# barry-mir/mixing-style-transfer

Hardware: AMD Instinct MI355X
Metric: triplets/sec (10 s @ 44.1 kHz, 4-stem, bs=24) (higher is better)
Workload: dtype f32

## Files before the change

### mixing-style-transfer_amd/csrc/fft_pk.h

```cpp
#pragma once
#include <hip/hip_runtime.h>

namespace mstpk {

typedef float v2f __attribute__((ext_vector_type(2)));
typedef float v4f __attribute__((ext_vector_type(4)));

__device__ __forceinline__ v2f mk(float x, float y) {
  v2f r;
  r.x = x, r.y = y;
  return r;
}
__device__ __forceinline__ v2f add_mi(v2f a, v2f b) {
  v2f d;
  asm("v_pk_add_f32 %0, %1, %2 op_sel:[0,1] op_sel_hi:[1,0] neg_hi:[0,1]" : "=v"(d) : "v"(a), "v"(b));
  return d;
}
__device__ __forceinline__ v2f sub_mi(v2f a, v2f b) {
  v2f d;
  asm("v_pk_add_f32 %0, %1, %2 op_sel:[0,1] op_sel_hi:[1,0] neg_lo:[0,1]" : "=v"(d) : "v"(a), "v"(b));
  return d;
}
__device__ __forceinline__ v2f cmul(v2f a, v2f w) {
  v2f t, d;
// ... 32 lines not shown
  v[2] = add_mi(e2, o2);
  v[6] = sub_mi(e2, o2);
  v[3] = add_mi(e3, o3);
  v[7] = sub_mi(e3, o3);
}

__device__ __forceinline__ void dft16(v2f* x) {
  constexpr float c1 = 0.92387953251128675613f, s1 = 0.38268343236508977173f;
#pragma unroll
  for (int a = 0; a < 4; ++a) dft4(x[a], x[a + 4], x[a + 8], x[a + 12]);
  x[1 + 4] = cmul(x[1 + 4], mk(c1, -s1));
  x[1 + 8] = mul_w8(x[1 + 8]);
  x[1 + 12] = cmul(x[1 + 12], mk(s1, -c1));
  x[2 + 4] = mul_w8(x[2 + 4]);
  x[2 + 12] = mul_w8(x[2 + 12]);
  x[3 + 4] = cmul(x[3 + 4], mk(s1, -c1));
  x[3 + 8] = mul_w8(x[3 + 8]);
  x[3 + 12] = cmul(x[3 + 12], mk(-c1, s1));
  dft4(x[0], x[1], x[2], x[3]);
  dft4(x[4], x[5], x[6], x[7]);
  dft4<true, true>(x[8], x[9], x[10], x[11]);
  dft4<true, false>(x[12], x[13], x[14], x[15]);
}

constexpr int kScr = 1152;
constexpr int kTw2Rows = 7;
constexpr int kTw3Rows = 14;

__device__ __forceinline__ int jb_of(int lane) { return lane ? 128 - lane : 64; }

struct NoFill {
  __device__ __forceinline__ void operator()() const {}
};
template <class F1 = NoFill, class F2 = NoFill>
__device__ __forceinline__ void fft1024(v2f (&x)[16], v2f* scr, const v2f* tw2, const v2f* tw3, int lane, F1 fill1 = F1(),
                                        F2 fill2 = F2()) {
  dft16(x);
  {
    v4f* row = reinterpret_cast<v4f*>(scr + 18 * lane);
#pragma unroll
    for (int q = 0; q < 8; ++q) {
      v4f w;
      w.x = x[2 * q].x, w.y = x[2 * q].y, w.z = x[2 * q + 1].x, w.w = x[2 * q + 1].y;
      row[q] = w;
    }
  }
  __builtin_amdgcn_wave_barrier();
  {
    const int m = lane & 15;
    const v2f* src = scr + 18 * (lane >> 4) + (m >> 2) + 4 * (m & 3);
#pragma unroll
    for (int u = 0; u < 2; ++u)
#pragma unroll
      for (int t = 0; t < 8; ++t) x[8 * u + t] = src[72 * u + 144 * t];
    v2f w2[8];
#pragma unroll
    for (int t = 1; t < 8; ++t) w2[t] = tw2[(t - 1) * 64 + lane];
    fill1();
#pragma unroll
    for (int t = 1; t < 8; ++t) {
      x[t] = cmul(x[t], w2[t]);
      x[8 + t] = cmul(x[8 + t], w2[t]);
    }
    dft8(x);
    dft8(x + 8);
  }
  __builtin_amdgcn_wave_barrier();
  {
    v2f* dst = scr + 144 * (lane >> 4) + (lane & 15);
#pragma unroll
    for (int u = 0; u < 2; ++u)
#pragma unroll
      for (int t = 0; t < 8; ++t) dst[576 * u + 16 * t] = x[8 * u + t];
  }
  __builtin_amdgcn_wave_barrier();
  {
    const v2f* sa = scr + lane;
    const v2f* sb = scr + jb_of(lane);
#pragma unroll
    for (int t = 0; t < 8; ++t) x[t] = sa[144 * t], x[8 + t] = sb[144 * t];
    fill2();
#pragma unroll
    for (int t = 1; t < 8; ++t) {
      x[t] = cmul(x[t], tw3[(t - 1) * 64 + lane]);
      x[8 + t] = cmul(x[8 + t], tw3[(7 + t - 1) * 64 + lane]);
    }
    dft8(x);
    dft8(x + 8);
  }
}

inline void fill_twiddles_host(float2* tw2, float2* tw3) {
  const double pi = 3.14159265358979323846;
  for (int t = 1; t < 8; ++t)
    for (int lane = 0; lane < 64; ++lane) {
      const double a = -2.0 * pi * (double)((lane & 15) * t) / 128.0;
      tw2[(t - 1) * 64 + lane] = make_float2((float)cos(a), (float)sin(a));
      for (int u = 0; u < 2; ++u) {
        const int j = u ? (lane ? 128 - lane : 64) : lane;
        const double b = -2.0 * pi * (double)(j * t) / 1024.0;
        tw3[(u * 7 + t - 1) * 64 + lane] = make_float2((float)cos(b), (float)sin(b));
      }
    }
}

}
```

### mixing-style-transfer_amd/csrc/melfeat.hip

```cpp
#include "common.h"
#include "fft_wave.h"
#include "fft_pk.h"
#include "stage_a_tables.h"

#include <algorithm>
#include <cmath>
#include <memory>
#include <vector>


namespace {

constexpr int kWaves = 8;
constexpr int kFPW = 2;
constexpr int kTF = kWaves * kFPW;
constexpr int kTileStride = kTF + 1;
constexpr int kThreads = kWaves * 64;
constexpr int nf_of(int n_fft) { return n_fft >= 2048 ? 1 : kFPW; }
constexpr int kNumScalars = 80;

enum : int {
  S_LOGSUM = 0,
  S_LINSUM = 4,
  S_MASK = 8,
// ... 970 lines not shown
}

template <int NFFT, int NB, typename ST>
int launch_melfeat(const KParams& kp, int grid, hipStream_t st) {
  return launch_stage_a<melfeat_kernel<NFFT, NB, ST>>(kp, grid, kThreads, GenericLds<NFFT>::bytes(kp.tw_count, kp.tw2_count, kp.nnz, kp.M, kp.tile_bufs), st);
}
template <int NFFT, typename ST, int WPS>
int launch_melfeat_spw(const KParams& kp, int grid, hipStream_t st) {
  return launch_stage_a<melfeat_spw_kernel<NFFT, ST, WPS>>(kp, grid, SpwGeom<WPS>::THREADS, SpwLds<NFFT, WPS>::bytes(kp.tw2_count, kp.nnz, kp.M), st);
}

#include "melfeat_v2.inc"
#include "melfeat_v2_2048.inc"

}

static_assert(sizeof(stage_a::F2) == sizeof(float2), "stage_a_tables.h's pairs are uploaded as float2");

struct mst_plan {
  int sr, n_fft, hop, n_mels, detailed_bins, feat_dim;
  int batches_per_run;
  mst::DevBuf<float> window;
  struct {
    int nb, nnz, tw_count, tw2_count, glen[4], goff[4];
    mst::DevBuf<float2> tw, tw2, post;
    mst::DevBuf<float> melw;
    mst::DevBuf<LaneBand> lanebands;
  } gen;
  struct {
    bool ok = false;
    int wps = 3;
    int nslot = 0, maxcnt = 0, segw_count = 0, glen[kV2Slots] = {0}, goff[kV2Slots] = {0};
    mst::DevBuf<float2> tw2, tw3, tw4, segw;
    mst::DevBuf<int> start, id, bandtab;
  } sw;
};

namespace {

struct StageAEnv {
  int batches_per_run, spw_wps;
  bool v2_wps2, generic, v2_nostd;
  bool old_kernels;
};
StageAEnv read_stage_a_env() {
  auto num = [](const char* name, int dflt) { const char* e = getenv(name); return e ? atoi(e) : dflt; };
  const char* a = getenv("MST_STAGE_A");
  StageAEnv s;
  s.batches_per_run = getenv("MST_MELFEAT_BATCHES") ? std::max(1, num("MST_MELFEAT_BATCHES", 0)) : 0;
  s.spw_wps = num("MST_SPW_WPS", 3);
  s.v2_wps2 = num("MST_V2_WPS", 0) == 2, s.generic = getenv("MST_MELFEAT_GENERIC"), s.v2_nostd = getenv("MST_V2_NOSTD");
  s.old_kernels = s.generic || (a && (!strcmp(a, "spw") || !strcmp(a, "generic")));
  return s;
}

int frames_per_run_of(const mst_plan* p, int F) {
  if (p->batches_per_run > 0) return p->batches_per_run * kTF;
  int fpr = (F + 31) / 32;
  fpr += fpr & 1;
  return std::max(2 * kTF, fpr);
}
int runs_per_clip(const mst_plan* p, int F) {
  const int fpr = frames_per_run_of(p, F);
  return (F + fpr - 1) / fpr;
}
int pstride_of(const mst_plan* p) { return 4 * p->n_mels + kNumScalars; }
// ... 22 lines not shown
  MST_REQUIRE(hop >= 1 && n_mels >= 4 && n_mels <= 256, "mst_plan_create: bad hop=%d / n_mels=%d", hop, n_mels);
  MST_REQUIRE(detailed_bins >= 0 && detailed_bins <= 256 && (detailed_bins == 0 || detailed_bins < n_mels ||
              detailed_bins == n_mels), "mst_plan_create: bad detailed_bins=%d", detailed_bins);
  std::unique_ptr<mst_plan> p(new mst_plan());
  p->sr = sample_rate, p->n_fft = n_fft, p->hop = hop, p->n_mels = n_mels, p->detailed_bins = detailed_bins;
  const int sd = detailed_bins > 0 ? detailed_bins + 2 : 5;
  p->feat_dim = 4 * (10 + sd) + 4;
  const StageAEnv env = read_stage_a_env();
  p->batches_per_run = env.batches_per_run;
  const int n_bins = n_fft / 2 + 1;
  auto& g = p->gen;
  auto& sw = p->sw;
  const bool v2 = n_fft == 1024 && hop == 256, v4 = n_fft == 2048 && hop == 512 && n_mels <= 128;
  sw.wps = (env.v2_wps2 || n_mels > 128 || v4) ? 2 : 3;
  stage_a::PieceTable t;
  if (v2 || v4) t = stage_a::build_pieces(fb, n_bins, n_mels, v2 ? stage_a::v2_piece_opts(n_mels) : stage_a::v4_piece_opts());
  sw.ok = t.ok, sw.nslot = t.nslot, sw.maxcnt = t.maxcnt, sw.segw_count = (int)t.segw.size();
  for (int r = 0; r < kV2Slots; ++r) sw.glen[r] = t.glen[r], sw.goff[r] = t.goff[r];
  const std::vector<int> bands = !t.ok ? std::vector<int>() : v2 ? stage_a::pack_bands16(t, n_mels, stage_a::kV2Dump) : stage_a::pack_bands8(t, n_mels);
  std::vector<float2> t2(mstpk::kTw2Rows * 64), t3(mstpk::kTw3Rows * 64);
  mstpk::fill_twiddles_host(t2.data(), t3.data());
  const std::vector<stage_a::F2> t4 = v4 ? stage_a::tw4_twiddles() : std::vector<stage_a::F2>();

  g.nb = n_mels <= 128 ? 2 : 4;
  const stage_a::LaneBandTable lb = stage_a::build_lane_bands(fb, n_bins, n_mels, g.nb);
  g.nnz = lb.nnz;
  for (int r = 0; r < 4; ++r) g.glen[r] = lb.glen[r], g.goff[r] = lb.goff[r];
  const std::vector<stage_a::F2> tw = stage_a::fft_twiddles(n_fft / 2), post = stage_a::post_twiddles(n_fft);
  std::vector<stage_a::F2> tw2;
  if (n_fft <= 1024) tw2 = stage_a::fft_twiddles(n_fft);
  g.tw_count = (int)tw.size(), g.tw2_count = (int)tw2.size();
  if (tw2.empty()) tw2.push_back(stage_a::F2{1.f, 0.f});
  auto f2 = [](const std::vector<stage_a::F2>& v) { return reinterpret_cast<const float2*>(v.data()); };
  int rc;
  if ((t.ok && ((rc = sw.tw2.upload(t2.data(), t2.size())) || (rc = sw.tw3.upload(t3.data(), t3.size())) ||
                (v4 && (rc = sw.tw4.upload(f2(t4), t4.size()))) || (rc = sw.segw.upload(f2(t.segw), t.segw.size())) ||
                (rc = sw.start.upload(t.start.data(), t.start.size())) || (rc = sw.id.upload(t.id.data(), t.id.size())) ||
                (rc = sw.bandtab.upload(bands.data(), bands.size())))) ||
      (rc = p->window.upload(window, (size_t)n_fft)) || (rc = g.tw.upload(f2(tw), tw.size())) || (rc = g.tw2.upload(f2(tw2), tw2.size())) ||
      (rc = g.post.upload(f2(post), post.size())) || (rc = g.melw.upload(lb.melw.data(), lb.melw.size())) ||
      (rc = g.lanebands.upload(lb.lanebands.data(), lb.lanebands.size())))
    return rc;
  *out = p.release();
  return MST_OK;
}

void mst_plan_destroy(mst_plan* p) { delete p; }

int mst_plan_frames(const mst_plan* p, int T) { return p ? 1 + T / p->hop : MST_EINVAL; }
int mst_plan_feature_dim(const mst_plan* p) { return p ? p->feat_dim : MST_EINVAL; }

size_t mst_melfeat_workspace_bytes(const mst_plan* p, int B, int T) {
  if (!p || B <= 0 || T <= 0) return 0;
  const int F = 1 + T / p->hop;
  const int runs = std::max(runs_per_clip(p, F), p->sw.ok ? sw_runs(p, F) : 0);
  return mst::align_up((size_t)B * runs * pstride_of(p) * sizeof(float), 256);
}

}

namespace {

struct LogmelOut {
  int layout = MST_LOGMEL_REF;
  void* lo = nullptr;
  unsigned* absmax = nullptr;
};

bool plan_uses_v2(const mst_plan* p) { return p->sw.ok && !read_stage_a_env().old_kernels; }

template <typename Fn>
int with_sample_type(bool pcm16, Fn fn) { return pcm16 ? fn(short{}) : fn(float{}); }
template <typename Fn>
auto with_n_fft(int n_fft, Fn fn) {
  if (n_fft == 512) return fn(std::integral_constant<int, 512>{});
  if (n_fft == 1024) return fn(std::integral_constant<int, 1024>{});
  return fn(std::integral_constant<int, 2048>{});
}

template <typename Params, typename Launch>
int launch_sliding_window(const mst_plan* p, Params& k, const LogmelOut& lmo, bool pcm16, Launch launch) {
  const auto& sw = p->sw;
  k.out_mode = lmo.layout, k.logmel_lo = lmo.lo, k.absmax = lmo.absmax;
  k.tw2 = sw.tw2.get(), k.tw3 = sw.tw3.get(), k.segw = sw.segw.get();
  k.nslot = sw.nslot, k.segw_count = sw.segw_count, k.maxcnt = sw.maxcnt, k.fpw = sw_fpw(p, k.F);
  for (size_t r = 0; r < std::size(k.glen); ++r) k.glen[r] = sw.glen[r], k.goff[r] = sw.goff[r];
  return with_sample_type(pcm16, launch);
}

int launch_v2_2048(const mst_plan* p, K4Params k, const LogmelOut& lmo, bool pcm16, hipStream_t st) {
  k.tw4 = p->sw.tw4.get(), k.pstart = p->sw.start.get(), k.pid = p->sw.id.get(), k.bandtab = p->sw.bandtab.get();
  return launch_sliding_window(p, k, lmo, pcm16, [&](auto s) { return launch_melfeat_v2_2048<decltype(s)>(k, k.B * k.runs_per_clip, st); });
}

int launch_v2(const mst_plan* p, K2Params k, const LogmelOut& lmo, bool pcm16, bool no_std, hipStream_t st) {
  k.segstart = p->sw.start.get(), k.segid = p->sw.id.get(), k.bandtab = reinterpret_cast<const int2*>(p->sw.bandtab.get());
  const bool stdt = v2_table_is_standard(p) && !no_std;
  return launch_sliding_window(p, k, lmo, pcm16, [&](auto s) {
    using ST = decltype(s);
    const int grid = k.B * k.runs_per_clip;
    if (p->n_mels > 128) return launch_melfeat_v2<ST, 2, 4>(k, grid, st);
    return p->sw.wps == 3 ? launch_melfeat_v2<ST, 3>(k, grid, st, stdt) : launch_melfeat_v2<ST, 2>(k, grid, st);
  });
}

size_t generic_lds_bytes(const mst_plan* p, int tile_bufs) {
  return with_n_fft(p->n_fft, [&](auto N) { return GenericLds<N()>::bytes(p->gen.tw_count, p->gen.tw2_count, p->gen.nnz, p->n_mels, tile_bufs); });
}

int launch_generic_or_spw(const mst_plan* p, KParams kp, bool pcm16, const StageAEnv& env, hipStream_t st) {
  const auto& g = p->gen;
  kp.tw = g.tw.get(), kp.tw2 = g.tw2.get(), kp.post = g.post.get(), kp.melw = g.melw.get(), kp.lanebands = g.lanebands.get();
  kp.hop = p->hop, kp.tw_count = g.tw_count, kp.tw2_count = g.tw2_count, kp.nnz = g.nnz;
  for (int r = 0; r < 4; ++r) kp.glen[r] = g.glen[r], kp.goff[r] = g.goff[r];
  kp.frames_per_run = frames_per_run_of(p, kp.F);
  bool base16 = true;
  for (int i = 0; i < 4; ++i) base16 = base16 && (reinterpret_cast<uintptr_t>(kp.stem[i]) & 15) == 0;
  kp.vec_ok = base16 && (kp.T % 2 == 0) && (p->hop % 2 == 0) && (kp.clip_stride % 2 == 0);
  kp.vec4_ok = base16 && (kp.T % 4 == 0) && (p->hop % 4 == 0) && (kp.clip_stride % 4 == 0);
  kp.tile_bufs = generic_lds_bytes(p, 2) <= kMaxLds ? 2 : 1;
  const int grid = kp.B * kp.runs_per_clip, n_fft = p->n_fft, M = p->n_mels;
  const bool spw_ok = kp.vec_ok && kp.vec4_ok && p->hop * 4 == n_fft && M <= 128 && g.nb == 2 && (n_fft == 512 || n_fft == 1024) && !env.generic;
  const bool spw3 = spw_ok && env.spw_wps == 3 && n_fft == 1024 && SpwLds<1024, 3>::bytes(g.tw2_count, g.nnz, M) <= kMaxLds;
  const bool spw2 = spw_ok && !spw3 &&
                    (n_fft == 1024 ? SpwLds<1024, 2>::bytes(g.tw2_count, g.nnz, M) : SpwLds<512, 2>::bytes(g.tw2_count, g.nnz, M)) <= kMaxLds;
  return with_sample_type(pcm16, [&](auto s) {
    using ST = decltype(s);
    if (spw3) return launch_melfeat_spw<1024, ST, 3>(kp, grid, st);
    if (spw2) return n_fft == 1024 ? launch_melfeat_spw<1024, ST, 2>(kp, grid, st) : launch_melfeat_spw<512, ST, 2>(kp, grid, st);
// ... 102 lines not shown
```

### mixing-style-transfer_amd/csrc/melfeat_v2.inc

```

constexpr int kV2Slots = 6;

struct K2Params {
  const void* stem[4];
  long long clip_stride;
  float* logmel;
  void* logmel_lo;
  unsigned* absmax;
  int out_mode;
  float* partials;
  const float* window;
  const float2* tw2;
  const float2* tw3;
  const float2* segw;
  const int* segstart;
  const int* segid;
  const int2* bandtab;
  int B, T, F, M;
  int nslot, glen[kV2Slots], goff[kV2Slots], segw_count;
  int maxcnt;
  int fpw;
  int runs_per_clip, pstride;
};

namespace v2 {
using namespace mstpk;

constexpr int kP2 = 0;
constexpr int kExN = 288;
constexpr int kExDump = kExN - 1;
constexpr int kExHi = 544;
constexpr int kExLo = kExHi + kExN;
static_assert(kExLo + kExN <= kScr, "exchange areas must fit the FFT scratch");
static_assert(kExDump == stage_a::kV2Dump && kV2Slots == stage_a::kMaxSlots, "the piece table is built for these limits");

__device__ __forceinline__ v2f pair_power4(v2f zk, v2f zm) {
  const v2f s = zk + zm, d = zk - zm;
  const v2f q = s * s;
  v2f r;
  asm("v_pk_fma_f32 %0, %1, %1, %2 op_sel:[1,1,0] op_sel_hi:[0,0,1]" : "=v"(r) : "v"(d), "v"(q));
  return r;
}

__device__ __forceinline__ v2f sel2(unsigned long long m, v2f a, v2f b) {
  float rx, ry;
  const float ax = a.x, ay = a.y, bx = b.x, by = b.y;
  asm("v_cndmask_b32 %0, %1, %2, %3" : "=v"(rx) : "v"(bx), "v"(ax), "s"(m));
  asm("v_cndmask_b32 %0, %1, %2, %3" : "=v"(ry) : "v"(by), "v"(ay), "s"(m));
  return mk(rx, ry);
}

template <typename ST>
__device__ __forceinline__ float ld_at(const ST* base, int idx) {
  const unsigned boff = (unsigned)idx * (unsigned)sizeof(ST);
  return Smp<ST>::lds(reinterpret_cast<const ST*>(reinterpret_cast<const char*>(base) + boff));
}

__device__ __forceinline__ v2f bcast_fma(float w, v2f q, v2f acc) { return __builtin_elementwise_fma(mk(w, w), q, acc); }

typedef float f4u __attribute__((ext_vector_type(4), aligned(4)));

typedef float f32x4v __attribute__((ext_vector_type(4)));
typedef _Float16 h16x2 __attribute__((ext_vector_type(2)));

template <int NBL>
struct CmGeom {
  static constexpr int MB = 64 * NBL, PSTR = 2 * MB + 16, TILE = 4 * PSTR;
};
template <int NBL, int BLK>
__device__ __forceinline__ void block_absmax(const float (&out)[2 * NBL][BLK], int lane, int nv, int M, unsigned* s_amax) {
  float bm = 0.f;
#pragma unroll
  for (int r = 0; r < NBL; ++r)
#pragma unroll
    for (int e = 0; e < BLK; ++e)
      if (e < nv && lane + 64 * r < M) bm = fmaxf(bm, fmaxf(fabsf(out[2 * r][e]), fabsf(out[2 * r + 1][e])));
  bm = mst::wave_max(bm);
  if (lane == 0) atomicMax(s_amax, __float_as_uint(bm));
}
template <int NBL, int BLK, int WPS, int SCR>
__device__ __forceinline__ void cm_stage(const float (&out)[2 * NBL][BLK], v2f* s_scr, int h, int stem, int lane, int nv, int out_mode) {
  using G = CmGeom<NBL>;
  static_assert((BLK / 4) * G::TILE <= 2 * SCR, "the staged frames of a wave must fit its FFT scratch");
#pragma unroll
  for (int e = 0; e < BLK; ++e) {
    if (e < nv) {
      float* tl = reinterpret_cast<float*>(s_scr + ((e & 3) * WPS + h) * SCR) + (e >> 2) * G::TILE + stem * G::PSTR;
#pragma unroll
      for (int r = 0; r < NBL; ++r) {
        const float vL = out[2 * r][e], vR = out[2 * r + 1][e];
        v2f val;
// ... 36 lines not shown
          const int b = 64 * it + lane;
          v2f a[4];
#pragma unroll
          for (int j = 0; j < 4; ++j) a[j] = *reinterpret_cast<const v2f*>(tl + j * G::PSTR + 2 * b);
          if (b < M) {
            dhi[b] = f32x4v{a[0].x, a[1].x, a[2].x, a[3].x};
            if (logmel_lo) dlo[b] = f32x4v{a[0].y, a[1].y, a[2].y, a[3].y};
          }
        }
      }
    }
  }
}


}

template <int WPS> struct V2Geom {
  static constexpr int BLK = WPS == 2 ? 8 : 4;
  static constexpr int SB = BLK;
  static constexpr bool WIN_LDS = true;
  static constexpr bool MIX_EARLY = WPS == 2;
};

template <int WPS, int NBL>
struct V2Lds {
  static constexpr int BLK = NBL == 2 ? V2Geom<WPS>::BLK : 4, MB = 64 * NBL, WAVES = 4 * WPS;
  static constexpr int tw2 = 0, tw3 = tw2 + mstpk::kTw2Rows * 64 * 8, segw = tw3 + mstpk::kTw3Rows * 64 * 8;
  static constexpr int a_win = 0, a_exch = a_win + (V2Geom<WPS>::WIN_LDS ? 1024 * 4 : 0);
  static constexpr int a_scr = a_exch + WPS * BLK * 4 * MB * 4, a_amax = a_scr + WAVES * mstpk::kScr * 8;
  static constexpr size_t bytes(int segw_count) { return (size_t)segw + (size_t)segw_count * 8 + a_amax + 16; }
  static_assert(WAVES * NBL * 64 + WAVES * 16 <= 2 * WAVES * mstpk::kScr, "the reduction buffer must fit the FFT scratch");
};

template <typename ST, int WPS, int NBL = 2, bool CM = false, bool STD = false>
__global__ __launch_bounds__(WPS * 256) void melfeat_v2_kernel(const K2Params p) {
#pragma clang fp contract(off)
  using namespace mstpk;
  using namespace v2;
  using L = V2Lds<WPS, NBL>;
  constexpr int kWaves = L::WAVES, kThreads = kWaves * 64, BLK = L::BLK, MB = L::MB;
  constexpr bool kUnrollBlock = STD && BLK == 4;
  constexpr bool WIN_LDS = V2Geom<WPS>::WIN_LDS, MIX_EARLY = V2Geom<WPS>::MIX_EARLY;
  constexpr int SB = BLK;
  constexpr float kLn2 = 0.69314718055994530942f;
  extern __shared__ __attribute__((aligned(16))) unsigned char smem[];
  v2f* s_tw2 = reinterpret_cast<v2f*>(smem + L::tw2);
  v2f* s_tw3 = reinterpret_cast<v2f*>(smem + L::tw3);
  v2f* s_segw = reinterpret_cast<v2f*>(smem + L::segw);
  unsigned char* after_segw = reinterpret_cast<unsigned char*>(s_segw + p.segw_count);
  float* s_win = reinterpret_cast<float*>(after_segw + L::a_win);
  float* s_exch = reinterpret_cast<float*>(after_segw + L::a_exch);
  v2f* s_scr = reinterpret_cast<v2f*>(after_segw + L::a_scr);
  unsigned* s_amax = reinterpret_cast<unsigned*>(after_segw + L::a_amax);
  static_assert(!STD || NBL == 2, "the standard table has 128 bands");
  const int M = STD ? 128 : p.M, T = p.T;
  const int nslot = STD ? 3 : p.nslot, maxcnt = STD ? 1 : p.maxcnt;
  constexpr int kStdLen[3] = {14, 3, 0}, kStdOff[3] = {0, 14, 17};
  constexpr bool cm = CM;

  const int tid = threadIdx.x, lane = tid & 63;
  const int wave = __builtin_amdgcn_readfirstlane(tid >> 6);
  const int work = mst::xcd_remap(blockIdx.x, gridDim.x);
  const int clip = work / p.runs_per_clip, run = work % p.runs_per_clip;
  const int fpr = WPS * p.fpw;
  const int f_begin = run * fpr;
  const int f_end = min(p.F, f_begin + fpr);
  {
    const v2f* g2 = reinterpret_cast<const v2f*>(p.tw2);
    const v2f* g3 = reinterpret_cast<const v2f*>(p.tw3);
    const v2f* gs = reinterpret_cast<const v2f*>(p.segw);
    for (int i = tid; i < kTw2Rows * 64; i += kThreads) s_tw2[i] = g2[i];
    for (int i = tid; i < kTw3Rows * 64; i += kThreads) s_tw3[i] = g3[i];
    for (int i = tid; i < p.segw_count; i += kThreads) s_segw[i] = gs[i];
    if (WIN_LDS)
      for (int i = tid; i < 1024; i += kThreads) s_win[i] = p.window[i];
    if (tid == 0) *s_amax = 0u;
  }
  const int stem = wave / WPS, h = wave % WPS;
  auto chan = [&](int c) {
    return static_cast<const ST*>(p.stem[c >> 1]) + (size_t)clip * p.clip_stride + (size_t)(c & 1) * T;
  };
  const ST* const xL = chan(2 * stem);
  const ST* const xR = chan(2 * stem + 1);
  const int o_begin = f_begin * 256;
  const int o_end = (f_end == p.F) ? T : min(T, f_end * 256);
  const int o_piv = min(o_begin, T - 1);
  const float pvL = Smp<ST>::ld(xL + o_piv), pvR = Smp<ST>::ld(xR + o_piv);
  v2f* scr = s_scr + wave * kScr;
  float* exch = s_exch + h * (BLK * 4 * MB);

  v2f wp[8];
#pragma unroll
  for (int q = 0; q < 8; ++q)
    wp[q] = WIN_LDS ? mk(0.f, 0.f) : mk(p.window[lane + 64 * (2 * q)], p.window[lane + 64 * (2 * q + 1)]);
  constexpr int NSL = NBL == 2 ? 3 : kV2Slots;
  int seg_start[NSL], seg_id[NSL];
#pragma unroll
  for (int r = 0; r < NSL; ++r) {
    seg_start[r] = r < nslot ? p.segstart[r * 64 + lane] : 0;
    seg_id[r] = r < nslot ? p.segid[r * 64 + lane] : kExDump;
  }
  int2 btab[NBL];
#pragma unroll
  for (int r = 0; r < NBL; ++r) btab[r] = p.bandtab[r * 64 + lane];
  const int jb = jb_of(lane);
  const bool l0 = lane == 0;

  float acc_db[NBL], acc_log = 0.f, acc_lin = 0.f, acc_mask = 0.f, mixsq = 0.f;
// ... 166 lines not shown
    for (int w = 0; w < WPS; ++w) {
      const float* a = red2 + (WPS * s + w) * 16;
#pragma unroll
      for (int k = 0; k < 13; ++k) v[k] += a[k];
      pk0 = fmaxf(pk0, a[13]), pk1 = fmaxf(pk1, a[14]);
    }
    float* q = part + 4 * M;
    q[S_LOGSUM + s] = v[0];
    q[S_LINSUM + s] = v[1];
    q[S_SQ + 2 * s] = v[2], q[S_SQ + 2 * s + 1] = v[3];
    q[S_DSUM + 2 * s] = v[4], q[S_DSUM + 2 * s + 1] = v[5];
    q[S_DSQ + 2 * s] = v[6], q[S_DSQ + 2 * s + 1] = v[7];
    q[S_CROSS + s] = v[8];
    q[S_MID + s] = v[9];
    q[S_SIDE + s] = v[10];
    q[S_MASK + s] = v[12];
    q[S_PEAK + 2 * s] = pk0, q[S_PEAK + 2 * s + 1] = pk1;
    q[S_PIVOT + 2 * s] = Smp<ST>::ld(chan(2 * s) + o_piv), q[S_PIVOT + 2 * s + 1] = Smp<ST>::ld(chan(2 * s + 1) + o_piv);
  }
  if (cm && p.absmax && tid == 0) atomicMax(p.absmax + clip, *s_amax);
  if (tid == 8) {
    float mxs = 0.f;
    for (int w = 0; w < kWaves; ++w) mxs += red2[w * 16 + 11];
    part[4 * M + S_MIX] = mxs;
    part[4 * M + S_NSAMP] = (float)max(0, o_end - o_begin);
    part[4 * M + S_NFRAME] = (float)max(0, f_end - f_begin);
  }
}

template <typename ST, int WPS, int NBL = 2>
int launch_melfeat_v2(const K2Params& kp, int grid, hipStream_t st, bool std_table = false) {
  const size_t lds = V2Lds<WPS, NBL>::bytes(kp.segw_count);
  if constexpr (WPS == 3 && NBL == 2)
    if (std_table && kp.out_mode != 0) return launch_stage_a<melfeat_v2_kernel<ST, WPS, NBL, true, true>>(kp, grid, WPS * 256, lds, st);
  return kp.out_mode != 0 ? launch_stage_a<melfeat_v2_kernel<ST, WPS, NBL, true>>(kp, grid, WPS * 256, lds, st)
                          : launch_stage_a<melfeat_v2_kernel<ST, WPS, NBL, false>>(kp, grid, WPS * 256, lds, st);
}
```

### mixing-style-transfer_amd/csrc/melfeat_v2_frame.inc

```
{
      constexpr bool STATIC = MST_FRAME_STATIC != 0;
      constexpr int R = STATIC ? (MST_FRAME_STATIC ? (MST_FRAME_I) : 0) & 3 : 0;
      constexpr int SLOT = STATIC ? (MST_FRAME_STATIC ? (MST_FRAME_I) : 0) % SB : 0;
      const int i = (MST_FRAME_I);
      const int f = f0 + blk * BLK + i;
      v2f x[16];
      float ma = 0.f, mb = 0.f;
#pragma unroll
      for (int t = 0; t < 16; ++t) {
        v2f w;
        if (WIN_LDS) {
          const float wv = s_win[lane + 64 * t];
          w = mk(wv, wv);
        } else {
          w = (t & 1) ? __builtin_shufflevector(wp[t >> 1], wp[t >> 1], 1, 1)
                      : __builtin_shufflevector(wp[t >> 1], wp[t >> 1], 0, 0);
        }
        x[t] = raw[(t + 4 * R) & 15] * w;
        ma = fmaxf(ma, fabsf(x[t].x)), mb = fmaxf(mb, fabsf(x[t].y));
      }
      const unsigned ua = wave_umax_uniform(__float_as_uint(ma)), ub = wave_umax_uniform(__float_as_uint(mb));
      const bool more = blk * BLK + i + 1 < nfw;
      v2f nxt[4];
      {
        const int base2 = f * 256 + 512, b2 = base2 + lane;
        if (more) {
          if (base2 + 255 < T) {
#pragma unroll
            for (int j = 0; j < 4; ++j)
              nxt[j] = mk(ld_at(xL, b2 + 64 * j), ld_at(xR, b2 + 64 * j));
          } else {
#pragma unroll
            for (int j = 0; j < 4; ++j) nxt[j] = ld2(b2 + 64 * j);
          }
        } else {
#pragma unroll
          for (int j = 0; j < 4; ++j) nxt[j] = mk(0.f, 0.f);
        }
      }
      float mx[8];
      const bool mix_on = blk * BLK + i + kMixLead < nfw;
      const int mp = mix_on ? (f + kMixLead) * 256 + 64 * stem + lane : T;
      if (MIX_EARLY) {
        const int q = min(mp, T - 1);
// ... 3 lines not shown
      int sh = 0;
      if (ua != 0u && ub != 0u) sh = max(-40, min(40, (int)(ua >> 23) - (int)(ub >> 23)));
      if (sh != 0) {
        const float sc = __uint_as_float((unsigned)(127 + sh) << 23);
#pragma unroll
        for (int t = 0; t < 16; ++t) x[t].y *= sc;
      }
      const float ia = ua != 0u ? 1.0f : 0.f;
      const float ib = ub != 0u ? __uint_as_float((unsigned)(127 - 2 * sh) << 23) : 0.f;
      auto moments = [&]() __attribute__((always_inline)) {
#pragma unroll
        for (int j = 0; j < 4; ++j) {
          const bool mk_ = f * 256 + lane + 64 * j < T;
          const float L = mk_ ? raw[(8 + j + 4 * R) & 15].x : 0.f, Rr = mk_ ? raw[(8 + j + 4 * R) & 15].y : 0.f;
          const float dL = mk_ ? L - pvL : 0.f, dR = mk_ ? Rr - pvR : 0.f;
          sqL = fmaf(L, L, sqL), sqR = fmaf(Rr, Rr, sqR);
          pkL = fmaxf(pkL, fabsf(L)), pkR = fmaxf(pkR, fabsf(Rr));
          dsL += dL, dsR += dR;
          dqL = fmaf(dL, dL, dqL), dqR = fmaf(dR, dR, dqR);
          cr = fmaf(dL, dR, cr);
          mid = fmaf(L + Rr, L + Rr, mid);
          side = fmaf(L - Rr, L - Rr, side);
        }
      };
      auto mixture = [&]() __attribute__((always_inline)) {
        if (mp < T) {
          const float mL = ((mx[0] + mx[2]) + mx[4]) + mx[6];
          const float mR = ((mx[1] + mx[3]) + mx[5]) + mx[7];
          mixsq = fmaf(mL, mL, mixsq);
          mixsq = fmaf(mR, mR, mixsq);
        }
      };
      if (!MIX_EARLY) {
        fft1024(x, scr, s_tw2, s_tw3, lane, moments);
      } else {
        fft1024(x, scr, s_tw2, s_tw3, lane, moments, mixture);
      }
      if (!MIX_EARLY) {
        const int q = min(mp, T - 1);
#pragma unroll
        for (int c = 0; c < 8; ++c) mx[c] = ld_at(chan(c), q);
      }
      {
        const v2f sc4 = mk(0.25f * ia, 0.25f * ib);
        v2f* P2 = scr + kP2;
#pragma unroll
        for (int t = 0; t < 4; ++t) {
          const v2f zm_a = sel2(1ull, x[(8 - t) & 7], x[15 - t]);
          const v2f zm_b = sel2(1ull, x[15 - t], x[7 - t]);
          P2[lane + 128 * t] = pair_power4(x[t], zm_a) * sc4;
          P2[jb + 128 * t] = pair_power4(x[8 + t], zm_b) * sc4;
        }
        if (l0) P2[512] = x[4] * x[4] * mk(ia, ib);
        if (lane < 16) P2[513 + lane] = mk(0.f, 0.f);
      }
      __builtin_amdgcn_wave_barrier();
      auto walk_slot = [&](auto rc) __attribute__((always_inline)) {
        constexpr int r = decltype(rc)::value;
        if (r < NSL && r < nslot) {
          v2f slo = mk(0.f, 0.f), shi = mk(0.f, 0.f);
          const v2f* pw = s_segw + (STD ? kStdOff[r < 3 ? r : 0] : p.goff[r < NSL ? r : 0]) * 64 + lane;
          const v2f* pp = scr + kP2 + seg_start[r < NSL ? r : 0];
          if constexpr (STD) {
            constexpr int N = kStdLen[r < 3 ? r : 0], CH = 7;
#pragma unroll
            for (int k0 = 0; k0 < N; k0 += CH) {
              v2f wv[CH], qv[CH];
#pragma unroll
              for (int k = 0; k < CH; ++k)
                if (k0 + k < N) wv[k] = pw[(k0 + k) * 64], qv[k] = pp[k0 + k];
#pragma unroll
              for (int k = 0; k < CH; ++k)
                if (k0 + k < N) slo = bcast_fma(wv[k].x, qv[k], slo), shi = bcast_fma(wv[k].y, qv[k], shi);
            }
          } else {
            const int n = p.glen[r < NSL ? r : 0];
#pragma unroll 2
            for (int k = 0; k < n; ++k) {
              const v2f w = pw[k * 64];
              const v2f q = pp[k];
              slo = bcast_fma(w.x, q, slo);
              shi = bcast_fma(w.y, q, shi);
            }
          }
          scr[kExHi + seg_id[r < NSL ? r : 0]] = shi;
          scr[kExLo + seg_id[r < NSL ? r : 0]] = slo;
        }
      };
      walk_slot(std::integral_constant<int, 0>()), walk_slot(std::integral_constant<int, 1>()), walk_slot(std::integral_constant<int, 2>());
      walk_slot(std::integral_constant<int, 3>()), walk_slot(std::integral_constant<int, 4>()), walk_slot(std::integral_constant<int, 5>());
      static_assert(NSL <= 6, "walk_slot is spelled out for six slots");
      __builtin_amdgcn_wave_barrier();
#pragma unroll
      for (int r = 0; r < NBL; ++r) {
        const int b = lane + 64 * r;
        v2f m;
// ... 42 lines not shown
```

### mixing-style-transfer_amd/csrc/stage_a_tables.h

```cpp
#pragma once
#include <algorithm>
#include <cmath>
#include <vector>

namespace stage_a {

struct F2 { float x, y; };
struct LaneBand { int band, start; };
inline F2 unit(double a) { return F2{(float)std::cos(a), (float)std::sin(a)}; }

inline std::vector<F2> fft_twiddles(int NC) {
  static const int kPasses[3][5][2] = {{{4, 1}, {4, 4}, {4, 16}, {4, 64}}, {{8, 1}, {8, 8}, {8, 64}}, {{8, 1}, {8, 8}, {4, 64}, {4, 256}}};
  std::vector<F2> tw;
  if (NC != 256 && NC != 512 && NC != 1024) return tw;
  for (const int* pass = kPasses[NC / 512][0]; pass[0]; pass += 2) {
    const int R = pass[0], NS = pass[1];
    if (NS == 1) continue;
    const int nbf = NS <= 64 ? 1 : NC / R / 64;
    for (int u = 0; u < nbf; ++u)
      for (int t = 1; t < R; ++t)
        for (int lane = 0; lane < 64; ++lane) tw.push_back(unit(-2.0 * M_PI * (double)((lane + 64 * u) % NS * t) / (double)(NS * R)));
  }
  return tw;
}
// ... 114 lines not shown
  t.nslot = (np + 63) / 64;
  if (np > o.dump || t.nslot > o.max_slots) return t;
  t.start.assign((size_t)t.nslot * 64, 0);
  t.id.assign((size_t)t.nslot * 64, o.dump);
  int off = 0;
  for (int r = 0; r < t.nslot; ++r) {
    int gl = 0;
    for (int lane = 0; lane < 64 && r * 64 + lane < np; ++lane) gl = std::max(gl, pieces[order[r * 64 + lane]].len);
    t.glen[r] = gl, t.goff[r] = off;
    t.segw.resize((size_t)(off + gl) * 64, F2{0.f, 0.f});
    for (int lane = 0; lane < 64 && r * 64 + lane < np; ++lane) {
      const Piece pc = pieces[order[r * 64 + lane]];
      t.start[(size_t)r * 64 + lane] = pc.start, t.id[(size_t)r * 64 + lane] = order[r * 64 + lane];
      for (int i = 0; i < pc.len; ++i) t.segw[(size_t)(off + i) * 64 + lane] = F2{wl[pc.start + i], wh[pc.start + i]};
    }
    off += gl;
  }
  t.segw.resize(std::max<size_t>(2, t.segw.size() + (t.segw.size() & 1)), F2{0.f, 0.f});
  t.ok = true;
  return t;
}

inline std::vector<int> pack_bands16(const PieceTable& t, int M, int dump) {
  std::vector<int> tab(2 * 256, dump);
  for (int b = 0; b < M; ++b) tab[2 * b] = t.first[b] | (t.cnt[b] << 16), tab[2 * b + 1] = t.first[b + 1] | (t.cnt[b + 1] << 16);
  return tab;
}
inline std::vector<int> pack_bands8(const PieceTable& t, int M) {
  std::vector<int> tab(128, 0);
  for (int b = 0; b < M; ++b) tab[b] = t.first[b] | (t.cnt[b] << 8) | (t.first[b + 1] << 16) | (t.cnt[b + 1] << 24);
  return tab;
}

}
```

Measured before the change: 2849.

## Store per-lane twiddle, window and segment-weight tables as padded LDS rows

The standard-table v2 kernel's LDS constants (FFT twiddles tw2/tw3, mel segment weights, window) are rearranged on the host so each lane's entries sit contiguously in an odd-16-byte-pitch row. The kernel can then load them with 128-bit LDS reads instead of many strided 64-bit or 32-bit reads. The segment-weight accumulation also switches to packed FMAs that select the low or high half of the weight pair. This cuts LDS instruction count but adds a new fixed LDS layout, a host table build, and a hard requirement that the row tables exist.

```diff
diff --git a/mixing-style-transfer_amd/csrc/fft_pk.h b/mixing-style-transfer_amd/csrc/fft_pk.h
--- a/mixing-style-transfer_amd/csrc/fft_pk.h
+++ b/mixing-style-transfer_amd/csrc/fft_pk.h
@@ -88,7 +88,7 @@
 struct NoFill {
   __device__ __forceinline__ void operator()() const {}
 };
-template <class F1 = NoFill, class F2 = NoFill>
+template <bool ROW2 = false, bool ROW3 = false, class F1 = NoFill, class F2 = NoFill>
 __device__ __forceinline__ void fft1024(v2f (&x)[16], v2f* scr, const v2f* tw2, const v2f* tw3, int lane, F1 fill1 = F1(),
                                         F2 fill2 = F2()) {
   dft16(x);
@@ -110,8 +110,18 @@
 #pragma unroll
       for (int t = 0; t < 8; ++t) x[8 * u + t] = src[72 * u + 144 * t];
     v2f w2[8];
+    if constexpr (ROW2) {
+      const v4f* row = reinterpret_cast<const v4f*>(tw2);
 #pragma unroll
-    for (int t = 1; t < 8; ++t) w2[t] = tw2[(t - 1) * 64 + lane];
+      for (int q = 0; q < 3; ++q) {
+        const v4f w = row[q];
+        w2[2 * q + 1] = mk(w.x, w.y), w2[2 * q + 2] = mk(w.z, w.w);
+      }
+      w2[7] = tw2[6];
+    } else {
+#pragma unroll
+      for (int t = 1; t < 8; ++t) w2[t] = tw2[(t - 1) * 64 + lane];
+    }
     fill1();
 #pragma unroll
     for (int t = 1; t < 8; ++t) {
@@ -136,10 +146,21 @@
 #pragma unroll
     for (int t = 0; t < 8; ++t) x[t] = sa[144 * t], x[8 + t] = sb[144 * t];
     fill2();
+    if constexpr (ROW3) {
+      const v4f* row = reinterpret_cast<const v4f*>(tw3);
 #pragma unroll
-    for (int t = 1; t < 8; ++t) {
-      x[t] = cmul(x[t], tw3[(t - 1) * 64 + lane]);
-      x[8 + t] = cmul(x[8 + t], tw3[(7 + t - 1) * 64 + lane]);
+      for (int q = 0; q < 7; ++q) {
+        const v4f w = row[q];
+        const int a = 2 * q < 7 ? 2 * q + 1 : 2 * q + 2, b = 2 * q + 1 < 7 ? 2 * q + 2 : 2 * q + 3;
+        x[a] = cmul(x[a], mk(w.x, w.y));
+        x[b] = cmul(x[b], mk(w.z, w.w));
+      }
+    } else {
+#pragma unroll
+      for (int t = 1; t < 8; ++t) {
+        x[t] = cmul(x[t], tw3[(t - 1) * 64 + lane]);
+        x[8 + t] = cmul(x[8 + t], tw3[(7 + t - 1) * 64 + lane]);
+      }
     }
     dft8(x);
     dft8(x + 8);
diff --git a/mixing-style-transfer_amd/csrc/melfeat.hip b/mixing-style-transfer_amd/csrc/melfeat.hip
--- a/mixing-style-transfer_amd/csrc/melfeat.hip
+++ b/mixing-style-transfer_amd/csrc/melfeat.hip
@@ -1026,6 +1026,7 @@
     int wps = 3;
     int nslot = 0, maxcnt = 0, segw_count = 0, glen[kV2Slots] = {0}, goff[kV2Slots] = {0};
     mst::DevBuf<float2> tw2, tw3, tw4, segw;
+    mst::DevBuf<float> rows;
     mst::DevBuf<int> start, id, bandtab;
   } sw;
 };
@@ -1114,11 +1115,14 @@
   g.tw_count = (int)tw.size(), g.tw2_count = (int)tw2.size();
   if (tw2.empty()) tw2.push_back(stage_a::F2{1.f, 0.f});
   auto f2 = [](const std::vector<stage_a::F2>& v) { return reinterpret_cast<const float2*>(v.data()); };
+  std::vector<float> rows;
+  if (v2 && t.ok && v2_table_is_standard(p.get()))
+    rows = stage_a::build_v2_rows(window, reinterpret_cast<const stage_a::F2*>(t2.data()), reinterpret_cast<const stage_a::F2*>(t3.data()), t.segw.data());
   int rc;
-  if ((t.ok && ((rc = sw.tw2.upload(t2.data(), t2.size())) || (rc = sw.tw3.upload(t3.data(), t3.size())) ||
+  if ((t.ok && ((!rows.empty() && (rc = sw.rows.upload(rows.data(), rows.size()))) || ((rc = sw.tw2.upload(t2.data(), t2.size())) || (rc = sw.tw3.upload(t3.data(), t3.size())) ||
                 (v4 && (rc = sw.tw4.upload(f2(t4), t4.size()))) || (rc = sw.segw.upload(f2(t.segw), t.segw.size())) ||
                 (rc = sw.start.upload(t.start.data(), t.start.size())) || (rc = sw.id.upload(t.id.data(), t.id.size())) ||
-                (rc = sw.bandtab.upload(bands.data(), bands.size())))) ||
+                (rc = sw.bandtab.upload(bands.data(), bands.size()))))) ||
       (rc = p->window.upload(window, (size_t)n_fft)) || (rc = g.tw.upload(f2(tw), tw.size())) || (rc = g.tw2.upload(f2(tw2), tw2.size())) ||
       (rc = g.post.upload(f2(post), post.size())) || (rc = g.melw.upload(lb.melw.data(), lb.melw.size())) ||
       (rc = g.lanebands.upload(lb.lanebands.data(), lb.lanebands.size())))
@@ -1176,7 +1180,7 @@
 }
 
 int launch_v2(const mst_plan* p, K2Params k, const LogmelOut& lmo, bool pcm16, bool no_std, hipStream_t st) {
-  k.segstart = p->sw.start.get(), k.segid = p->sw.id.get(), k.bandtab = reinterpret_cast<const int2*>(p->sw.bandtab.get());
+  k.segstart = p->sw.start.get(), k.segid = p->sw.id.get(), k.rows = p->sw.rows.get(), k.bandtab = reinterpret_cast<const int2*>(p->sw.bandtab.get());
   const bool stdt = v2_table_is_standard(p) && !no_std;
   return launch_sliding_window(p, k, lmo, pcm16, [&](auto s) {
     using ST = decltype(s);
diff --git a/mixing-style-transfer_amd/csrc/melfeat_v2.inc b/mixing-style-transfer_amd/csrc/melfeat_v2.inc
--- a/mixing-style-transfer_amd/csrc/melfeat_v2.inc
+++ b/mixing-style-transfer_amd/csrc/melfeat_v2.inc
@@ -15,6 +15,7 @@
   const float2* segw;
   const int* segstart;
   const int* segid;
+  const float* rows;
   const int2* bandtab;
   int B, T, F, M;
   int nslot, glen[kV2Slots], goff[kV2Slots], segw_count;
@@ -57,6 +58,17 @@
 }
 
 __device__ __forceinline__ v2f bcast_fma(float w, v2f q, v2f acc) { return __builtin_elementwise_fma(mk(w, w), q, acc); }
+
+__device__ __forceinline__ v2f bcast_fma_lo(v2f w, v2f q, v2f acc) {
+  v2f d;
+  asm("v_pk_fma_f32 %0, %1, %2, %3 op_sel_hi:[0,1,1]" : "=v"(d) : "v"(w), "v"(q), "v"(acc));
+  return d;
+}
+__device__ __forceinline__ v2f bcast_fma_hi(v2f w, v2f q, v2f acc) {
+  v2f d;
+  asm("v_pk_fma_f32 %0, %1, %2, %3 op_sel:[1,0,0] op_sel_hi:[1,1,1]" : "=v"(d) : "v"(w), "v"(q), "v"(acc));
+  return d;
+}
 
 typedef float f4u __attribute__((ext_vector_type(4), aligned(4)));
 
@@ -159,6 +171,35 @@
   static constexpr size_t bytes(int segw_count) { return (size_t)segw + (size_t)segw_count * 8 + a_amax + 16; }
   static_assert(WAVES * NBL * 64 + WAVES * 16 <= 2 * WAVES * mstpk::kScr, "the reduction buffer must fit the FFT scratch");
 };
+
+#ifndef MST_ROW_WIN
+#define MST_ROW_WIN 1
+#endif
+#ifndef MST_ROW_TW2
+#define MST_ROW_TW2 1
+#endif
+#ifndef MST_ROW_TW3
+#define MST_ROW_TW3 1
+#endif
+#ifndef MST_ROW_SEGW
+#define MST_ROW_SEGW 1
+#endif
+#ifndef MST_ROW_SEGW_CH
+#define MST_ROW_SEGW_CH 8
+#endif
+struct V2LdsStd {
+  using R = stage_a::V2Rows;
+  using B = V2Lds<3, 2>;
+  static constexpr int kSegw = 17 * 64;
+  static constexpr int tw2 = 0, tw3 = tw2 + (MST_ROW_TW2 ? 64 * R::pTw2 * 4 : mstpk::kTw2Rows * 64 * 8);
+  static constexpr int segw = tw3 + (MST_ROW_TW3 ? 64 * R::pTw3 * 4 : mstpk::kTw3Rows * 64 * 8);
+  static constexpr int win = segw + (MST_ROW_SEGW ? 64 * R::pSegw * 4 : kSegw * 8);
+  static constexpr int exch = win + (MST_ROW_WIN ? 64 * R::pWin * 4 : 1024 * 4);
+  static constexpr int scr = exch + (B::a_scr - B::a_exch), amax = scr + (B::a_amax - B::a_scr);
+  static constexpr size_t bytes() { return (size_t)amax + 16; }
+  static_assert(V2Geom<3>::WIN_LDS && tw3 % 16 == 0 && segw % 16 == 0 && win % 16 == 0 && exch % 16 == 0, "rows are 16-byte aligned");
+};
+static_assert(V2LdsStd::bytes() <= kMaxLds, "the row-form layout must pass launch_stage_a's 160 KiB limit");
 
 template <typename ST, int WPS, int NBL = 2, bool CM = false, bool STD = false>
 __global__ __launch_bounds__(WPS * 256) void melfeat_v2_kernel(const K2Params p) {
@@ -172,21 +213,28 @@
   constexpr int SB = BLK;
   constexpr float kLn2 = 0.69314718055994530942f;
   extern __shared__ __attribute__((aligned(16))) unsigned char smem[];
-  v2f* s_tw2 = reinterpret_cast<v2f*>(smem + L::tw2);
-  v2f* s_tw3 = reinterpret_cast<v2f*>(smem + L::tw3);
-  v2f* s_segw = reinterpret_cast<v2f*>(smem + L::segw);
-  unsigned char* after_segw = reinterpret_cast<unsigned char*>(s_segw + p.segw_count);
-  float* s_win = reinterpret_cast<float*>(after_segw + L::a_win);
-  float* s_exch = reinterpret_cast<float*>(after_segw + L::a_exch);
-  v2f* s_scr = reinterpret_cast<v2f*>(after_segw + L::a_scr);
-  unsigned* s_amax = reinterpret_cast<unsigned*>(after_segw + L::a_amax);
-  static_assert(!STD || NBL == 2, "the standard table has 128 bands");
+  static_assert(!STD || (WPS == 3 && NBL == 2 && CM), "the standard-table build is the 12-wave channel-minor one (V2LdsStd)");
+  using LS = V2LdsStd;
+  using RW = stage_a::V2Rows;
+  constexpr bool ROW_WIN = STD && MST_ROW_WIN, ROW_TW2 = STD && MST_ROW_TW2, ROW_TW3 = STD && MST_ROW_TW3, ROW_SEGW = STD && MST_ROW_SEGW;
+  unsigned char* after_segw = smem + L::segw + (size_t)p.segw_count * 8;
+  v2f* t_tw2 = reinterpret_cast<v2f*>(smem + (STD ? LS::tw2 : L::tw2));
+  v2f* t_tw3 = reinterpret_cast<v2f*>(smem + (STD ? LS::tw3 : L::tw3));
+  v2f* t_segw = reinterpret_cast<v2f*>(smem + (STD ? LS::segw : L::segw));
+  float* t_win = reinterpret_cast<float*>(STD ? smem + LS::win : after_segw + L::a_win);
+  float* s_exch = reinterpret_cast<float*>(STD ? smem + LS::exch : after_segw + L::a_exch);
+  v2f* s_scr = reinterpret_cast<v2f*>(STD ? smem + LS::scr : after_segw + L::a_scr);
+  unsigned* s_amax = reinterpret_cast<unsigned*>(STD ? smem + LS::amax : after_segw + L::a_amax);
   const int M = STD ? 128 : p.M, T = p.T;
   const int nslot = STD ? 3 : p.nslot, maxcnt = STD ? 1 : p.maxcnt;
   constexpr int kStdLen[3] = {14, 3, 0}, kStdOff[3] = {0, 14, 17};
   constexpr bool cm = CM;
 
   const int tid = threadIdx.x, lane = tid & 63;
+  const v2f* s_tw2 = ROW_TW2 ? reinterpret_cast<const v2f*>(reinterpret_cast<const float*>(t_tw2) + lane * RW::pTw2) : t_tw2;
+  const v2f* s_tw3 = ROW_TW3 ? reinterpret_cast<const v2f*>(reinterpret_cast<const float*>(t_tw3) + lane * RW::pTw3) : t_tw3;
+  const v2f* s_segw = ROW_SEGW ? reinterpret_cast<const v2f*>(reinterpret_cast<const float*>(t_segw) + lane * RW::pSegw) : t_segw;
+  const float* s_win = ROW_WIN ? t_win + lane * RW::pWin : t_win;
   const int wave = __builtin_amdgcn_readfirstlane(tid >> 6);
   const int work = mst::xcd_remap(blockIdx.x, gridDim.x);
   const int clip = work / p.runs_per_clip, run = work % p.runs_per_clip;
@@ -197,11 +245,22 @@
     const v2f* g2 = reinterpret_cast<const v2f*>(p.tw2);
     const v2f* g3 = reinterpret_cast<const v2f*>(p.tw3);
     const v2f* gs = reinterpret_cast<const v2f*>(p.segw);
-    for (int i = tid; i < kTw2Rows * 64; i += kThreads) s_tw2[i] = g2[i];
-    for (int i = tid; i < kTw3Rows * 64; i += kThreads) s_tw3[i] = g3[i];
-    for (int i = tid; i < p.segw_count; i += kThreads) s_segw[i] = gs[i];
-    if (WIN_LDS)
-      for (int i = tid; i < 1024; i += kThreads) s_win[i] = p.window[i];
+    auto rows_in = [&](void* dst, int off, int pitch) {
+      const v4f* g = reinterpret_cast<const v4f*>(p.rows + off);
+      for (int i = tid; i < 16 * pitch; i += kThreads) reinterpret_cast<v4f*>(dst)[i] = g[i];
+    };
+    if (ROW_TW2) rows_in(t_tw2, RW::oTw2, RW::pTw2);
+    else
+      for (int i = tid; i < kTw2Rows * 64; i += kThreads) t_tw2[i] = g2[i];
+    if (ROW_TW3) rows_in(t_tw3, RW::oTw3, RW::pTw3);
+    else
+      for (int i = tid; i < kTw3Rows * 64; i += kThreads) t_tw3[i] = g3[i];
+    if (ROW_SEGW) rows_in(t_segw, RW::oSegw, RW::pSegw);
+    else
+      for (int i = tid; i < p.segw_count; i += kThreads) t_segw[i] = gs[i];
+    if (ROW_WIN) rows_in(t_win, RW::oWin, RW::pWin);
+    else if (WIN_LDS)
+      for (int i = tid; i < 1024; i += kThreads) t_win[i] = p.window[i];
     if (tid == 0) *s_amax = 0u;
   }
   const int stem = wave / WPS, h = wave % WPS;
@@ -434,7 +493,10 @@
 int launch_melfeat_v2(const K2Params& kp, int grid, hipStream_t st, bool std_table = false) {
   const size_t lds = V2Lds<WPS, NBL>::bytes(kp.segw_count);
   if constexpr (WPS == 3 && NBL == 2)
-    if (std_table && kp.out_mode != 0) return launch_stage_a<melfeat_v2_kernel<ST, WPS, NBL, true, true>>(kp, grid, WPS * 256, lds, st);
+    if (std_table && kp.out_mode != 0) {
+      MST_REQUIRE(kp.rows && kp.segw_count == V2LdsStd::kSegw, "mst_melfeat_forward: the standard-table build needs its row tables");
+      return launch_stage_a<melfeat_v2_kernel<ST, WPS, NBL, true, true>>(kp, grid, WPS * 256, V2LdsStd::bytes(), st);
+    }
   return kp.out_mode != 0 ? launch_stage_a<melfeat_v2_kernel<ST, WPS, NBL, true>>(kp, grid, WPS * 256, lds, st)
                           : launch_stage_a<melfeat_v2_kernel<ST, WPS, NBL, false>>(kp, grid, WPS * 256, lds, st);
 }
diff --git a/mixing-style-transfer_amd/csrc/melfeat_v2_frame.inc b/mixing-style-transfer_amd/csrc/melfeat_v2_frame.inc
--- a/mixing-style-transfer_amd/csrc/melfeat_v2_frame.inc
+++ b/mixing-style-transfer_amd/csrc/melfeat_v2_frame.inc
@@ -9,7 +9,11 @@
 #pragma unroll
       for (int t = 0; t < 16; ++t) {
         v2f w;
-        if (WIN_LDS) {
+        if constexpr (ROW_WIN) {
+          const v4f w4 = reinterpret_cast<const v4f*>(s_win)[t >> 2];
+          const float wv = w4[t & 3];
+          w = mk(wv, wv);
+        } else if (WIN_LDS) {
           const float wv = s_win[lane + 64 * t];
           w = mk(wv, wv);
         } else {
@@ -79,9 +83,9 @@
         }
       };
       if (!MIX_EARLY) {
-        fft1024(x, scr, s_tw2, s_tw3, lane, moments);
+        fft1024<ROW_TW2, ROW_TW3>(x, scr, s_tw2, s_tw3, lane, moments);
       } else {
-        fft1024(x, scr, s_tw2, s_tw3, lane, moments, mixture);
+        fft1024<ROW_TW2, ROW_TW3>(x, scr, s_tw2, s_tw3, lane, moments, mixture);
       }
       if (!MIX_EARLY) {
         const int q = min(mp, T - 1);
@@ -108,7 +112,28 @@
           v2f slo = mk(0.f, 0.f), shi = mk(0.f, 0.f);
           const v2f* pw = s_segw + (STD ? kStdOff[r < 3 ? r : 0] : p.goff[r < NSL ? r : 0]) * 64 + lane;
           const v2f* pp = scr + kP2 + seg_start[r < NSL ? r : 0];
-          if constexpr (STD) {
+          if constexpr (ROW_SEGW) {
+            constexpr int N = kStdLen[r < 3 ? r : 0], E0 = N ? kStdOff[r < 3 ? r : 0] : 0, CH = MST_ROW_SEGW_CH;
+            static_assert(E0 % 2 == 0 && CH % 2 == 0, "a 16-byte read holds an even entry and its successor");
+            const v4f* pr = reinterpret_cast<const v4f*>(s_segw) + E0 / 2;
+#pragma unroll
+            for (int k0 = 0; k0 < N; k0 += CH) {
+              v4f wv[CH / 2];
+              v2f qv[CH];
+#pragma unroll
+              for (int k = 0; k < CH; ++k) {
+                if (k0 + k < N && k % 2 == 0) wv[k / 2] = pr[(k0 + k) / 2];
+                if (k0 + k < N) qv[k] = pp[k0 + k];
+              }
+#pragma unroll
+              for (int k = 0; k < CH; ++k)
+                if (k0 + k < N) {
+                  const v4f w4 = wv[k / 2];
+                  const v2f w = k % 2 ? mk(w4.z, w4.w) : mk(w4.x, w4.y);
+                  slo = bcast_fma_lo(w, qv[k], slo), shi = bcast_fma_hi(w, qv[k], shi);
+                }
+            }
+          } else if constexpr (STD) {
             constexpr int N = kStdLen[r < 3 ? r : 0], CH = 7;
 #pragma unroll
             for (int k0 = 0; k0 < N; k0 += CH) {
diff --git a/mixing-style-transfer_amd/csrc/stage_a_tables.h b/mixing-style-transfer_amd/csrc/stage_a_tables.h
--- a/mixing-style-transfer_amd/csrc/stage_a_tables.h
+++ b/mixing-style-transfer_amd/csrc/stage_a_tables.h
@@ -170,4 +170,31 @@
   return tab;
 }
 
-}
+constexpr int row_pitch(int row_floats) {
+  const int units = (row_floats + 3) / 4;
+  return 4 * (units | 1);
+}
+inline std::vector<float> lane_rows(const float* tab, int n, int W) {
+  const int pitch = row_pitch(n * W);
+  std::vector<float> rows((size_t)64 * pitch, 0.f);
+  for (int lane = 0; lane < 64; ++lane)
+    for (int i = 0; i < n * W; ++i) rows[(size_t)lane * pitch + i] = tab[((size_t)(i / W) * 64 + lane) * W + i % W];
+  return rows;
+}
+struct V2Rows {
+  static constexpr int kTw2 = 2 * 7, kTw3 = 2 * 14, kSegw = 2 * 17, kWin = 16;
+  static constexpr int pTw2 = row_pitch(kTw2), pTw3 = row_pitch(kTw3), pSegw = row_pitch(kSegw), pWin = row_pitch(kWin);
+  static constexpr int oTw2 = 0, oTw3 = oTw2 + 64 * pTw2, oSegw = oTw3 + 64 * pTw3, oWin = oSegw + 64 * pSegw, kTotal = oWin + 64 * pWin;
+};
+inline std::vector<float> build_v2_rows(const float* window, const F2* tw2, const F2* tw3, const F2* segw) {
+  std::vector<float> all;
+  all.reserve(V2Rows::kTotal);
+  auto add = [&](const float* tab, int n, int W) {
+    const std::vector<float> r = lane_rows(tab, n, W);
+    all.insert(all.end(), r.begin(), r.end());
+  };
+  add(&tw2->x, 7, 2), add(&tw3->x, 14, 2), add(&segw->x, 17, 2), add(window, 16, 1);
+  return all;
+}
+
+}
```

Result: no change. 2859 (median of 6 runs) (+0.4%).
